# labRadioVision/federated

Hardware: AMD Instinct MI355X
Metric: device-resident GB/s, CFA reduce of K neighbour fp32 param buckets; 1/2/4/8 GPU (higher is better)
Workload: dtype f32

## Files before the change

### federated_amd/csrc/cfa_ring.hip

```cpp
#include <type_traits>

#include "cfa_internal.h"
#include "cfa_slide_shape.h"

namespace {

constexpr int kWinMaxDev = 8;
struct WindowArgs {
  const float* rows[kWinMaxDev + 8];
  float* out[kWinMaxDev];
  float a[kWinMaxDev];
  int nb;
};

template <int HL, int HR, typename Row>
__device__ __forceinline__ f4 ring_fold(Row row, float a) {
  f4 acc = row(HL);
#pragma unroll
  for (int j = 0; j < HL; ++j) acc = seq_step(acc, row(j), a);
#pragma unroll
  for (int j = 0; j < HR; ++j) acc = seq_step(acc, row(HL + 1 + j), a);
  return acc;
}

template <int HL, int HR, int U, bool SC1>
__device__ __forceinline__ void window_body(const WindowArgs& w, long long nvec) {
  constexpr int R = kWinMaxDev + HL + HR;
  constexpr long long kTile = (long long)kBlock * U;
  const int nr = w.nb + HL + HR;
  for (long long t = blockIdx.x; t * kTile < nvec; t += gridDim.x) {
    const long long base = t * kTile + threadIdx.x;
    f4 r[U][R];
#pragma unroll
    for (int k = 0; k < R; ++k)
      if (k < nr)
#pragma unroll
        for (int u = 0; u < U; ++u) {
          const long long i = base + (long long)u * kBlock;
          if (i < nvec) r[u][k] = ld4<true>(w.rows[k], i);
        }
#pragma unroll
    for (int b = 0; b < kWinMaxDev; ++b)
      if (b < w.nb) {
        const __amdgpu_buffer_rsrc_t o = out_rsrc(w.out[b], (unsigned)(nvec * 16));
#pragma unroll
        for (int u = 0; u < U; ++u) {
          const long long i = base + (long long)u * kBlock;
          if (i < nvec) {
            const f4 y = ring_fold<HL, HR>([&](int j) { return r[u][b + j]; }, w.a[b]);
            if constexpr (SC1)
              st16_buf<kStoreSc1>(o, i, y);
            else
              st4<true>(w.out[b], i, y);
          }
        }
      }
  }
}

template <int HL, int HR, int U, bool SC1>
__global__ __launch_bounds__(kBlock) void window_vec_kernel(WindowArgs w, long long nvec) {
  window_body<HL, HR, U, SC1>(w, nvec);
}

struct RingArgs {
  const float* in;
  float* out;
  const float* alphas;
  long long pitch;
  long long off;
  int D;
};

template <int HL, int HR, int U, bool SC1>
__global__ __launch_bounds__(kBlock) void ring_round_kernel(RingArgs ra, long long nvec) {
  const int p = blockIdx.y;
  WindowArgs w;
  w.nb = min(kWinMaxDev, ra.D - p * kWinMaxDev);
#pragma unroll
  for (int k = 0; k < kWinMaxDev + HL + HR; ++k) {
    const int g = ((p * kWinMaxDev - HL + k) % ra.D + ra.D) % ra.D;
    w.rows[k] = ra.in + (long long)g * ra.pitch + ra.off;
  }
#pragma unroll
  for (int b = 0; b < kWinMaxDev; ++b) {
    const int d = min(p * kWinMaxDev + b, ra.D - 1);
    w.out[b] = ra.out + (long long)d * ra.pitch + ra.off;
    w.a[b] = ra.alphas[d];
  }
  window_body<HL, HR, U, SC1>(w, nvec);
}

struct SlideArgs {
  const float* in;
  float* out;
  const float* alphas;
  long long in_pitch, out_pitch;
  long long off;
  int rows, first, count, seg;
};

template <int HL, int HR, int PF, int U, bool SC1>
__global__ __launch_bounds__(kBlock) void ring_slide_kernel(SlideArgs sa, long long nvec) {
  constexpr int W = HL + HR + 1;
  constexpr int RS = W + PF;
  constexpr long long kTile = (long long)kBlock * U;
  const int n0 = (int)blockIdx.y * sa.seg;
  const int len = min(sa.seg, sa.count - n0);
  const int total = len + HL + HR;
  const int d0 = sa.first + n0;
  int g0 = (d0 - HL) % sa.rows;
  if (g0 < 0) g0 += sa.rows;
  const int o0 = d0 >= sa.rows ? d0 - sa.rows : d0;
  const float* const in = sa.in + sa.off;
  float* const out = sa.out + sa.off;
  const float* const in_end = in + (long long)sa.rows * sa.in_pitch;
  float* const out_end = out + (long long)sa.rows * sa.out_pitch;
  for (long long t = blockIdx.x; t * kTile < nvec; t += gridDim.x) {
    const long long i = t * kTile + threadIdx.x;
    if (i >= nvec) continue;
    bool ok[U];
    unsigned voff[U];
#pragma unroll
    for (int v = 0; v < U; ++v) {
      ok[v] = i + (long long)v * kBlock < nvec;
      voff[v] = (unsigned)((ok[v] ? i + (long long)v * kBlock : i) * 16);
    }
    const float* rp = in + (long long)g0 * sa.in_pitch;
    float* op = out + (long long)o0 * sa.out_pitch;
    f4 r[RS][U];
    auto load_row = [&](f4(&slot)[U]) {
#pragma unroll
      for (int v = 0; v < U; ++v)
        slot[v] = __builtin_nontemporal_load(reinterpret_cast<const f4*>(reinterpret_cast<const char*>(rp) + voff[v]));
      rp += sa.in_pitch;
      if (rp == in_end) rp = in;
    };
#pragma unroll
    for (int q = 0; q < RS - 1; ++q)
      if (q < total) load_row(r[q]);
    for (int n = 0; n < len; n += RS) {
#pragma unroll
      for (int u = 0; u < RS; ++u) {
        const int m = n + u;
        if (m < len) {
          if (m + RS - 1 < total) load_row(r[(u + RS - 1) % RS]);
          const float a = sa.alphas[n0 + m];
          f4 acc[U];
#pragma unroll
          for (int v = 0; v < U; ++v) acc[v] = ring_fold<HL, HR>([&](int j) { return r[(u + j) % RS][v]; }, a);
#pragma unroll
          for (int v = 0; v < U; ++v)
            if (ok[v]) {
              if constexpr (SC1)
                st16_buf<kStoreSc1>(out_rsrc(op, (unsigned)(nvec * 16)), i + (long long)v * kBlock, acc[v]);
              else
                __builtin_nontemporal_store(acc[v], reinterpret_cast<f4*>(reinterpret_cast<char*>(op) + voff[v]));
            }
          op += sa.out_pitch;
          if (op == out_end) op = out;
        }
      }
    }
  }
}

__global__ __launch_bounds__(kBlock) void window_scalar_kernel(WindowArgs w, int hl, int hr,
                                                               long long begin, long long P) {
  for (long long i = begin + (long long)blockIdx.x * kBlock + threadIdx.x; i < P;
       i += (long long)gridDim.x * kBlock) {
    for (int b = 0; b < w.nb; ++b) {
      float acc = w.rows[b + hl][i];
      for (int j = 0; j < hl; ++j) acc = seq_step(acc, w.rows[b + j][i], w.a[b]);
      for (int j = 0; j < hr; ++j) acc = seq_step(acc, w.rows[b + hl + 1 + j][i], w.a[b]);
      w.out[b][i] = acc;
    }
  }
}

}

namespace {
struct WindowTune {
  int vec, sc1, blocks_per_cu;
};
static WindowTune window_tune() {
  WindowTune t{1, 0, 6};
  t.vec = env_int("CFA_WINDOW_VEC", t.vec) == 1 ? 1 : 2;
  t.sc1 = env_int("CFA_WINDOW_SC1", t.sc1) ? 1 : 0;
  t.blocks_per_cu = env_int("CFA_WINDOW_BLOCKS_PER_CU", t.blocks_per_cu);
  if (t.blocks_per_cu <= 0) t.blocks_per_cu = 2;
  return t;
}
static long long window_tiles(long long m, const WindowTune& t) {
  return (m + (long long)kBlock * t.vec - 1) / ((long long)kBlock * t.vec);
}
template <typename F>
void for_vec_sc1(const WindowTune& t, F&& fn) {
  using One = std::integral_constant<int, 1>;
  using Two = std::integral_constant<int, 2>;
  if (t.vec == 1) {
    if (t.sc1) fn(One{}, std::true_type{});
    else fn(One{}, std::false_type{});
  } else {
    if (t.sc1) fn(Two{}, std::true_type{});
    else fn(Two{}, std::false_type{});
  }
}
template <int HL, int HR>
void launch_window(const WindowArgs& w, long long nvec, hipStream_t st) {
  const WindowTune t = window_tune();
  const cfa_launch_t lc{t.blocks_per_cu, t.vec, 1};
  for_each_chunk(nvec, [&](long long done, long long m) {
    WindowArgs c = w;
    for (int k = 0; k < w.nb + HL + HR; ++k) c.rows[k] = w.rows[k] + done * 4;
    for (int b = 0; b < w.nb; ++b) c.out[b] = w.out[b] + done * 4;
    const unsigned grid = grid_for(window_tiles(m, t), lc);
    for_vec_sc1(t, [&](auto u, auto sc1) {
      window_vec_kernel<HL, HR, decltype(u)::value, decltype(sc1)::value><<<grid, kBlock, 0, st>>>(c, m);
    });
  });
}
template <int HL, int HR>
void launch_ring_round(const RingArgs& ra, long long nvec, hipStream_t st) {
  const WindowTune t = window_tune();
  const cfa_launch_t lc{t.blocks_per_cu, t.vec, 1};
  const unsigned passes = (unsigned)((ra.D + kWinMaxDev - 1) / kWinMaxDev);
  for_each_chunk(nvec, [&](long long done, long long m) {
    RingArgs c = ra;
    c.off = ra.off + done * 4;
    const long long tiles = window_tiles(m, t);
    long long gx = (grid_for(tiles, lc) + passes - 1) / passes;
    if (gx < 1) gx = 1;
    if (gx > tiles) gx = tiles;
    const dim3 grid((unsigned)gx, passes);
    for_vec_sc1(t, [&](auto u, auto sc1) {
      ring_round_kernel<HL, HR, decltype(u)::value, decltype(sc1)::value><<<grid, kBlock, 0, st>>>(c, m);
    });
  });
}

static_assert(kSlideBlock == kBlock, "cfa_slide_shape.h counts tiles of kBlock lanes");
static SlideTune slide_tune() {
  const SlideTune d = kSlideDefault;
  SlideTune t{env_int("CFA_SLIDE_SEGMENTS", d.segments), env_int("CFA_SLIDE_WG_PER_CU", d.wg_per_cu),
              env_int("CFA_SLIDE_PF", d.pf), env_int("CFA_SLIDE_SC1", d.sc1) ? 1 : 0, env_int("CFA_SLIDE_U", 0)};
  if (t.segments <= 0) t.segments = d.segments;
  if (t.wg_per_cu <= 0) t.wg_per_cu = d.wg_per_cu;
  if (t.pf < 1 || t.pf > 2) t.pf = d.pf;
  if (t.u != 1 && t.u != 2 && t.u != 4) t.u = 0;
  return t;
}
template <int HL, int HR, int PF, int U>
void launch_slide_shape(const SlideArgs& c, long long m, dim3 grid, bool sc1, hipStream_t st) {
  if (sc1) ring_slide_kernel<HL, HR, PF, U, true><<<grid, kBlock, 0, st>>>(c, m);
  else ring_slide_kernel<HL, HR, PF, U, false><<<grid, kBlock, 0, st>>>(c, m);
}
template <int HL, int HR, int U>
void launch_slide_u(const SlideArgs& c, long long m, dim3 grid, const SlideTune& t, hipStream_t st) {
  switch (t.pf) {
    case 1: launch_slide_shape<HL, HR, 1, U>(c, m, grid, t.sc1, st); break;
    default: launch_slide_shape<HL, HR, 2, U>(c, m, grid, t.sc1, st); break;
  }
}
template <int HL, int HR>
void launch_ring_slide(const SlideArgs& sa, long long nvec, hipStream_t st) {
  const SlideTune t = slide_tune();
  int segments = t.segments < sa.count ? t.segments : sa.count;
  if (segments > 65535) segments = 65535;
  SlideArgs c = sa;
  c.seg = (sa.count + segments - 1) / segments;
  const unsigned gy = (unsigned)((sa.count + c.seg - 1) / c.seg);
  for_each_chunk(nvec, [&](long long done, long long m) {
    c.off = done * 4;
    const int u = t.u ? t.u : slide_pick_u(m, kSlideDefault.u, device_cus(), t.wg_per_cu);
    const dim3 grid(shared_grid_x(slide_tiles(m, u), t.wg_per_cu, gy), gy);
    switch (u) {
      case 4: launch_slide_u<HL, HR, 4>(c, m, grid, t, st); break;
      case 2: launch_slide_u<HL, HR, 2>(c, m, grid, t, st); break;
      default: launch_slide_u<HL, HR, 1>(c, m, grid, t, st); break;
    }
  });
}

#define CFA_HLHR_ROW(F, L) {&F<L, 0>, &F<L, 1>, &F<L, 2>, &F<L, 3>, &F<L, 4>}
#define CFA_HLHR_TABLE(F) \
  {CFA_HLHR_ROW(F, 0), CFA_HLHR_ROW(F, 1), CFA_HLHR_ROW(F, 2), CFA_HLHR_ROW(F, 3), CFA_HLHR_ROW(F, 4)}
void (*const kWindowLaunch[5][5])(const WindowArgs&, long long, hipStream_t) = CFA_HLHR_TABLE(launch_window);
void (*const kRingLaunch[5][5])(const RingArgs&, long long, hipStream_t) = CFA_HLHR_TABLE(launch_ring_round);
void (*const kSlideLaunch[5][5])(const SlideArgs&, long long, hipStream_t) = CFA_HLHR_TABLE(launch_ring_slide);
#undef CFA_HLHR_TABLE
#undef CFA_HLHR_ROW
}

extern "C" int cfa_mix_window_f32(float* const* out, const float* const* rows, const float* alphas,
                                  int nb, int hl, int hr, size_t P, void* stream) {
  if (nb < 1 || nb > kWinMaxDev) return fail(CFA_E_INVALID, "nb %d outside 1..%d", nb, kWinMaxDev);
  if (hl < 0 || hr < 0 || hl > 4 || hr > 4) return fail(CFA_E_INVALID, "window %d/%d outside 0..4", hl, hr);
  if (!out || !rows || !alphas) return fail(CFA_E_INVALID, "null table");
  if (P == 0) return CFA_OK;
  WindowArgs w{};
  w.nb = nb;
  const int nr = nb + hl + hr;
  bool aligned = true;
  for (int k = 0; k < nr; ++k) {
    if (!rows[k]) return fail(CFA_E_INVALID, "null row %d", k);
    w.rows[k] = rows[k];
    aligned = aligned && (addr(rows[k]) & 15) == 0;
  }
  for (int b = 0; b < nb; ++b) {
    if (!out[b]) return fail(CFA_E_INVALID, "null output %d", b);
    for (int k = 0; k < nr; ++k)
      if (out[b] == rows[k]) return fail(CFA_E_INVALID, "output %d aliases row %d", b, k);
    w.out[b] = out[b];
    aligned = aligned && (addr(out[b]) & 15) == 0;
    w.a[b] = alphas[b];
  }
  hipStream_t st = (hipStream_t)stream;
  const long long nvec = aligned ? (long long)(P / 4) : 0;
  if (nvec > 0) {
    kWindowLaunch[hl][hr](w, nvec, st);
    if (int rc = check_launch("window_vec")) return rc;
  }
  const long long begin = nvec * 4;
  if (begin < (long long)P) {
    const long long len = (long long)P - begin;
    window_scalar_kernel<<<grid_for((len + kBlock - 1) / kBlock), kBlock, 0, st>>>(w, hl, hr, begin, (long long)P);
    if (int rc = check_launch("window_scalar")) return rc;
  }
  return CFA_OK;
}

extern "C" int cfa_mix_ring_round_f32(float* out, const float* in, size_t pitch, const float* alphas, int D,
                                      int hl, int hr, size_t P, void* stream) {
  if (D < 1) return fail(CFA_E_INVALID, "device count %d", D);
  if (hl < 0 || hr < 0 || hl > 4 || hr > 4) return fail(CFA_E_INVALID, "window %d/%d outside 0..4", hl, hr);
  if (hl + hr >= D) return fail(CFA_E_INVALID, "window %d/%d wider than %d devices", hl, hr, D);
  if (!out || !in || !alphas) return fail(CFA_E_INVALID, "null buffer");
  if (pitch < P) return fail(CFA_E_INVALID, "pitch %zu below P %zu", pitch, P);
  if (P == 0) return CFA_OK;
  if ((addr(out) & 15) || (addr(in) & 15) || (pitch % 4) || (P % 4))
    return fail(CFA_E_UNSUPPORTED, "ring round needs 16-byte aligned rows (pitch and P multiples of 4)");
  const long long outb = (long long)addr(out), inb = (long long)addr(in), span = (long long)D * (long long)pitch * 4;
  if (outb < inb + span && inb < outb + span) return fail(CFA_E_INVALID, "out overlaps in");
  if ((long long)(D + kWinMaxDev - 1) / kWinMaxDev > 65535) return fail(CFA_E_INVALID, "D=%d exceeds grid.y", D);
  RingArgs ra{in, out, alphas, (long long)pitch, 0, D};
  kRingLaunch[hl][hr](ra, (long long)(P / 4), (hipStream_t)stream);
  return check_launch("ring_round");
}

extern "C" int cfa_mix_ring_slide_f32(float* out, size_t out_pitch, const float* in, size_t in_pitch,
                                      const float* alphas, int rows, int first, int count, int hl, int hr,
                                      size_t P, void* stream) {
  if (!out || !in || !alphas) return fail(CFA_E_INVALID, "null buffer");
  if (rows < 1 || count < 1) return fail(CFA_E_INVALID, "rows %d / count %d below 1", rows, count);
  if (first < 0 || first >= rows || count > rows || (count != rows && first > rows - count))
    return fail(CFA_E_INVALID, "devices %d..%d outside a ring of %d rows", first, first + count - 1, rows);
  if (hl < 0 || hr < 0 || hl > 4 || hr > 4) return fail(CFA_E_INVALID, "window %d/%d outside 0..4", hl, hr);
  if (hl + hr >= rows) return fail(CFA_E_INVALID, "window %d/%d wider than %d rows", hl, hr, rows);
  if (in_pitch < P || out_pitch < P)
    return fail(CFA_E_INVALID, "pitch %zu/%zu below P %zu", out_pitch, in_pitch, P);
  if (P == 0) return CFA_OK;
  const unsigned long long outb = addr(out), inb = addr(in);
  const unsigned long long out_span = ((unsigned long long)(rows - 1) * out_pitch + P) * 4;
  const unsigned long long in_span = ((unsigned long long)(rows - 1) * in_pitch + P) * 4;
  if (outb < inb + in_span && inb < outb + out_span) return fail(CFA_E_INVALID, "out overlaps in");
  if ((outb & 15) || (inb & 15) || (out_pitch % 4) || (in_pitch % 4) || (P % 4))
    return fail(CFA_E_UNSUPPORTED, "ring slide needs 16-byte aligned rows (pitches and P multiples of 4)");
  SlideArgs sa{in, out, alphas, (long long)in_pitch, (long long)out_pitch, 0, rows, first, count, count};
  kSlideLaunch[hl][hr](sa, (long long)(P / 4), (hipStream_t)stream);
  return check_launch("ring_slide");
}
```

### federated_amd/csrc/cfa_slide_shape.h

```cpp
#pragma once

constexpr int kSlideBlock = 256;

struct SlideTune {
  int segments, wg_per_cu, pf, sc1, u;
};
constexpr SlideTune kSlideDefault{1, 4, 2, 0, 4};

inline long long slide_tiles(long long nvec, int u) {
  const long long tile = (long long)kSlideBlock * u;
  return (nvec + tile - 1) / tile;
}

inline int slide_pick_u(long long nvec, int want, int cus, int wg_per_cu) {
  int u = want >= 4 ? 4 : (want >= 2 ? 2 : 1);
  while (u > 1 && slide_tiles(nvec, u) < (long long)cus * wg_per_cu) u >>= 1;
  return u;
}
```

Baseline: 25360.

## Pair forward and backward ring walks per tile on same XCD for L2 reuse

Adds a paired mode to the ring slide kernel. For each column tile, one workgroup walks the first half of the devices forward and a partner walks the second half backward, so the two share the boundary rows. The tile-to-workgroup mapping uses an XCD-aware shift so partners are meant to land on the same XCD and reuse the shared rows from L2 instead of reloading them from HBM. Paired loads switch from nontemporal to regular cached loads. This is on by default, applies only when the full ring runs as a single segment, and adds index arithmetic and possible grid rounding overhead.

```diff
diff --git a/federated_amd/csrc/cfa_ring.hip b/federated_amd/csrc/cfa_ring.hip
--- a/federated_amd/csrc/cfa_ring.hip
+++ b/federated_amd/csrc/cfa_ring.hip
@@ -98,25 +98,27 @@
   long long in_pitch, out_pitch;
   long long off;
   int rows, first, count, seg;
+  int pair;
 };
 
-template <int HL, int HR, int PF, int U, bool SC1>
-__global__ __launch_bounds__(kBlock) void ring_slide_kernel(SlideArgs sa, long long nvec) {
+template <int HL, int HR, int PF, int U, bool SC1, bool PAIRED, bool BACK>
+__device__ __forceinline__ void slide_walks(const SlideArgs& sa, long long nvec, unsigned tiles, unsigned items,
+                                            int n0, int len) {
   constexpr int W = HL + HR + 1;
   constexpr int RS = W + PF;
   constexpr long long kTile = (long long)kBlock * U;
-  const int n0 = (int)blockIdx.y * sa.seg;
-  const int len = min(sa.seg, sa.count - n0);
   const int total = len + HL + HR;
-  const int d0 = sa.first + n0;
-  int g0 = (d0 - HL) % sa.rows;
+  const int d0 = sa.first + n0 + (BACK ? len - 1 : 0);
+  int g0 = (BACK ? d0 + HR : d0 - HL) % sa.rows;
   if (g0 < 0) g0 += sa.rows;
   const int o0 = d0 >= sa.rows ? d0 - sa.rows : d0;
   const float* const in = sa.in + sa.off;
   float* const out = sa.out + sa.off;
   const float* const in_end = in + (long long)sa.rows * sa.in_pitch;
   float* const out_end = out + (long long)sa.rows * sa.out_pitch;
-  for (long long t = blockIdx.x; t * kTile < nvec; t += gridDim.x) {
+  for (unsigned w = blockIdx.x; w < items; w += gridDim.x) {
+    const unsigned t = PAIRED ? slide_item_tile(w, sa.pair - 1) : w;
+    if (t >= tiles) continue;
     const long long i = t * kTile + threadIdx.x;
     if (i >= nvec) continue;
     bool ok[U];
@@ -131,10 +133,17 @@
     f4 r[RS][U];
     auto load_row = [&](f4(&slot)[U]) {
 #pragma unroll
-      for (int v = 0; v < U; ++v)
-        slot[v] = __builtin_nontemporal_load(reinterpret_cast<const f4*>(reinterpret_cast<const char*>(rp) + voff[v]));
-      rp += sa.in_pitch;
-      if (rp == in_end) rp = in;
+      for (int v = 0; v < U; ++v) {
+        const f4* const p = reinterpret_cast<const f4*>(reinterpret_cast<const char*>(rp) + voff[v]);
+        slot[v] = PAIRED ? *p : __builtin_nontemporal_load(p);
+      }
+      if constexpr (BACK) {
+        if (rp == in) rp = in_end;
+        rp -= sa.in_pitch;
+      } else {
+        rp += sa.in_pitch;
+        if (rp == in_end) rp = in;
+      }
     };
 #pragma unroll
     for (int q = 0; q < RS - 1; ++q)
@@ -145,10 +154,11 @@
         const int m = n + u;
         if (m < len) {
           if (m + RS - 1 < total) load_row(r[(u + RS - 1) % RS]);
-          const float a = sa.alphas[n0 + m];
+          const float a = sa.alphas[n0 + (BACK ? len - 1 - m : m)];
           f4 acc[U];
 #pragma unroll
-          for (int v = 0; v < U; ++v) acc[v] = ring_fold<HL, HR>([&](int j) { return r[(u + j) % RS][v]; }, a);
+          for (int v = 0; v < U; ++v)
+            acc[v] = ring_fold<HL, HR>([&](int j) { return r[(u + (BACK ? W - 1 - j : j)) % RS][v]; }, a);
 #pragma unroll
           for (int v = 0; v < U; ++v)
             if (ok[v]) {
@@ -157,11 +167,32 @@
               else
                 __builtin_nontemporal_store(acc[v], reinterpret_cast<f4*>(reinterpret_cast<char*>(op) + voff[v]));
             }
-          op += sa.out_pitch;
-          if (op == out_end) op = out;
+          if constexpr (BACK) {
+            if (op == out) op = out_end;
+            op -= sa.out_pitch;
+          } else {
+            op += sa.out_pitch;
+            if (op == out_end) op = out;
+          }
         }
       }
     }
+  }
+}
+
+template <int HL, int HR, int PF, int U, bool SC1, bool PAIRED>
+__global__ __launch_bounds__(kBlock) void ring_slide_kernel(SlideArgs sa, long long nvec) {
+  const unsigned tiles = (unsigned)slide_tiles(nvec, U);
+  if constexpr (PAIRED) {
+    const unsigned items = (unsigned)slide_pair_items(tiles, sa.pair - 1);
+    const int fwd = slide_fwd_len(sa.count);
+    if (!slide_item_back(blockIdx.x, sa.pair - 1))
+      slide_walks<HL, HR, PF, U, SC1, true, false>(sa, nvec, tiles, items, 0, fwd);
+    else if (fwd < sa.count)
+      slide_walks<HL, HR, PF, U, SC1, true, true>(sa, nvec, tiles, items, fwd, sa.count - fwd);
+  } else {
+    const int n0 = (int)blockIdx.y * sa.seg;
+    slide_walks<HL, HR, PF, U, SC1, false, false>(sa, nvec, tiles, tiles, n0, min(sa.seg, sa.count - n0));
   }
 }
 
@@ -244,17 +275,24 @@
 static SlideTune slide_tune() {
   const SlideTune d = kSlideDefault;
   SlideTune t{env_int("CFA_SLIDE_SEGMENTS", d.segments), env_int("CFA_SLIDE_WG_PER_CU", d.wg_per_cu),
-              env_int("CFA_SLIDE_PF", d.pf), env_int("CFA_SLIDE_SC1", d.sc1) ? 1 : 0, env_int("CFA_SLIDE_U", 0)};
+              env_int("CFA_SLIDE_PF", d.pf), env_int("CFA_SLIDE_SC1", d.sc1) ? 1 : 0, env_int("CFA_SLIDE_U", 0),
+              env_int("CFA_SLIDE_PAIR", d.pair)};
   if (t.segments <= 0) t.segments = d.segments;
   if (t.wg_per_cu <= 0) t.wg_per_cu = d.wg_per_cu;
   if (t.pf < 1 || t.pf > 2) t.pf = d.pf;
   if (t.u != 1 && t.u != 2 && t.u != 4) t.u = 0;
+  if (t.pair < kSlidePairOff || t.pair > kSlidePairXcd) t.pair = d.pair;
   return t;
 }
 template <int HL, int HR, int PF, int U>
 void launch_slide_shape(const SlideArgs& c, long long m, dim3 grid, bool sc1, hipStream_t st) {
-  if (sc1) ring_slide_kernel<HL, HR, PF, U, true><<<grid, kBlock, 0, st>>>(c, m);
-  else ring_slide_kernel<HL, HR, PF, U, false><<<grid, kBlock, 0, st>>>(c, m);
+  if (c.pair) {
+    if (sc1) ring_slide_kernel<HL, HR, PF, U, true, true><<<grid, kBlock, 0, st>>>(c, m);
+    else ring_slide_kernel<HL, HR, PF, U, false, true><<<grid, kBlock, 0, st>>>(c, m);
+  } else {
+    if (sc1) ring_slide_kernel<HL, HR, PF, U, true, false><<<grid, kBlock, 0, st>>>(c, m);
+    else ring_slide_kernel<HL, HR, PF, U, false, false><<<grid, kBlock, 0, st>>>(c, m);
+  }
 }
 template <int HL, int HR, int U>
 void launch_slide_u(const SlideArgs& c, long long m, dim3 grid, const SlideTune& t, hipStream_t st) {
@@ -271,10 +309,15 @@
   SlideArgs c = sa;
   c.seg = (sa.count + segments - 1) / segments;
   const unsigned gy = (unsigned)((sa.count + c.seg - 1) / c.seg);
+  c.pair = sa.count == sa.rows && gy == 1 && t.pair != kSlidePairOff ? 1 + slide_pair_shift(t.pair) : 0;
   for_each_chunk(nvec, [&](long long done, long long m) {
     c.off = done * 4;
     const int u = t.u ? t.u : slide_pick_u(m, kSlideDefault.u, device_cus(), t.wg_per_cu);
-    const dim3 grid(shared_grid_x(slide_tiles(m, u), t.wg_per_cu, gy), gy);
+    dim3 grid(shared_grid_x(slide_tiles(m, u), t.wg_per_cu, gy), gy);
+    if (c.pair) {
+      const long long items = slide_pair_items(slide_tiles(m, u), c.pair - 1);
+      grid.x = (unsigned)slide_pair_grid(items, c.pair - 1, shared_grid_x(items, t.wg_per_cu, 1));
+    }
     switch (u) {
       case 4: launch_slide_u<HL, HR, 4>(c, m, grid, t, st); break;
       case 2: launch_slide_u<HL, HR, 2>(c, m, grid, t, st); break;
@@ -367,7 +410,7 @@
   if (outb < inb + in_span && inb < outb + out_span) return fail(CFA_E_INVALID, "out overlaps in");
   if ((outb & 15) || (inb & 15) || (out_pitch % 4) || (in_pitch % 4) || (P % 4))
     return fail(CFA_E_UNSUPPORTED, "ring slide needs 16-byte aligned rows (pitches and P multiples of 4)");
-  SlideArgs sa{in, out, alphas, (long long)in_pitch, (long long)out_pitch, 0, rows, first, count, count};
+  SlideArgs sa{in, out, alphas, (long long)in_pitch, (long long)out_pitch, 0, rows, first, count, count, 0};
   kSlideLaunch[hl][hr](sa, (long long)(P / 4), (hipStream_t)stream);
   return check_launch("ring_slide");
 }
diff --git a/federated_amd/csrc/cfa_slide_shape.h b/federated_amd/csrc/cfa_slide_shape.h
--- a/federated_amd/csrc/cfa_slide_shape.h
+++ b/federated_amd/csrc/cfa_slide_shape.h
@@ -2,12 +2,13 @@
 
 constexpr int kSlideBlock = 256;
 
+enum { kSlidePairOff = 0, kSlidePairNext = 1, kSlidePairXcd = 2 };
 struct SlideTune {
-  int segments, wg_per_cu, pf, sc1, u;
+  int segments, wg_per_cu, pf, sc1, u, pair;
 };
-constexpr SlideTune kSlideDefault{1, 4, 2, 0, 4};
+constexpr SlideTune kSlideDefault{1, 4, 2, 0, 4, kSlidePairXcd};
 
-inline long long slide_tiles(long long nvec, int u) {
+constexpr long long slide_tiles(long long nvec, int u) {
   const long long tile = (long long)kSlideBlock * u;
   return (nvec + tile - 1) / tile;
 }
@@ -17,3 +18,19 @@
   while (u > 1 && slide_tiles(nvec, u) < (long long)cus * wg_per_cu) u >>= 1;
   return u;
 }
+
+constexpr int kSlideXcdShift = 3;
+
+constexpr int slide_fwd_len(int count) { return (count + 1) / 2; }
+constexpr int slide_pair_shift(int pair) { return pair == kSlidePairXcd ? kSlideXcdShift : 0; }
+constexpr long long slide_pair_items(long long tiles, int shift) {
+  return ((tiles + (1LL << shift) - 1) >> shift) << (shift + 1);
+}
+constexpr unsigned slide_item_tile(unsigned w, int shift) {
+  return (w >> (shift + 1) << shift) | (w & ((1u << shift) - 1));
+}
+constexpr bool slide_item_back(unsigned w, int shift) { return (w >> shift) & 1; }
+constexpr long long slide_pair_grid(long long items, int shift, long long want) {
+  const long long g = want >> (shift + 1) << (shift + 1);
+  return g < (2LL << shift) ? (2LL << shift) : (g < items ? g : items);
+}
```

After: 25370 (median of 2 runs). No clear change (+0.0%).
